# sekulas/vRod

Measured on AMD Instinct MI355X. Metric: queries/sec + recall@10 vs CPU ref, 10M×768 cosine, batch=1024, 1/2/4/8 GPU, higher is better.
Workload: dtype bf16

## Files before the change

vrod_amd/csrc/kernels_mfma_w4.hip:

```cpp
#include "mfma_common.h"
#include "w4_steal.h"

namespace vrod {

#ifdef VROD_W4_CLK
__device__ unsigned long long g_w4_clk[8];
#define W4_CLK(...) __VA_ARGS__
#else
#define W4_CLK(...)
#endif

template <int BASE, bool ZERO>
__device__ __forceinline__ void w4_mfma1(const bf16x8& x, const bf16x8& y) {
    if constexpr (ZERO)
        asm volatile("v_mfma_f32_16x16x32_bf16 a[%c2:%c3], %0, %1, 0" ::"v"(x), "v"(y), "i"(BASE), "i"(BASE + 3) : "memory");
    else
        asm volatile("v_mfma_f32_16x16x32_bf16 a[%c2:%c3], %0, %1, a[%c2:%c3]" ::"v"(x), "v"(y), "i"(BASE), "i"(BASE + 3) : "memory");
}
template <int MH, int NH, bool ZERO, int G>
__device__ __forceinline__ void w4_mfma_group(const bf16x8 (&FA)[4][2], const bf16x8 (&FB)[4][2]) {
    static_for<0, 4>([&](auto ic) {
        constexpr int I = G * 4 + decltype(ic)::value;
        constexpr int kk = I / 16, mm = (I / 4) % 4, nn = I % 4;
        w4_mfma1<((MH * 4 + mm) * 8 + NH * 4 + nn) * 4, ZERO && kk == 0>(FA[mm][kk], FB[nn][kk]);
    });
}
template <int BASE>
__device__ __forceinline__ f32x4 w4_read_acc() {
    f32x4 v;
    asm volatile("v_accvgpr_read_b32 %0, a[%c4]\n\tv_accvgpr_read_b32 %1, a[%c5]\n\tv_accvgpr_read_b32 %2, a[%c6]\n\tv_accvgpr_read_b32 %3, a[%c7]"
                 : "=v"(v[0]), "=v"(v[1]), "=v"(v[2]), "=v"(v[3]) : "i"(BASE), "i"(BASE + 1), "i"(BASE + 2), "i"(BASE + 3));
    return v;
}

#ifndef W4_RD_STRIDE_S
#define W4_RD_STRIDE_S "36"
#endif
__device__ __forceinline__ f32x4 w4_read_acc_dyn(uint32_t t) {
    f32x4 v;
    uint32_t tmp;
#define W4_RD(T)                                                                                    \
    "v_accvgpr_read_b32 %0, a[4*" #T "]\n\tv_accvgpr_read_b32 %1, a[4*" #T "+1]\n\t"                \
    "v_accvgpr_read_b32 %2, a[4*" #T "+2]\n\tv_accvgpr_read_b32 %3, a[4*" #T "+3]\n\ts_branch .Lw4rd_e_%=\n\t"
#define W4_RD8(A, B, C, D, E, F, G, H) W4_RD(A) W4_RD(B) W4_RD(C) W4_RD(D) W4_RD(E) W4_RD(F) W4_RD(G) W4_RD(H)
    asm volatile("s_getpc_b64 vcc\n"
                 ".Lw4rd_a_%=:\n\t"
                 "s_mul_i32 %4, %5, " W4_RD_STRIDE_S "\n\t"
                 "s_add_u32 vcc_lo, vcc_lo, %4\n\t"
                 "s_addc_u32 vcc_hi, vcc_hi, 0\n\t"
                 "s_add_u32 vcc_lo, vcc_lo, .Lw4rd_t_%=-.Lw4rd_a_%=\n\t"
                 "s_addc_u32 vcc_hi, vcc_hi, 0\n\t"
                 "s_setpc_b64 vcc\n"
                 ".Lw4rd_t_%=:\n\t"
                 W4_RD8(0, 1, 2, 3, 4, 5, 6, 7) W4_RD8(8, 9, 10, 11, 12, 13, 14, 15)
                 W4_RD8(16, 17, 18, 19, 20, 21, 22, 23) W4_RD8(24, 25, 26, 27, 28, 29, 30, 31)
                 W4_RD8(32, 33, 34, 35, 36, 37, 38, 39) W4_RD8(40, 41, 42, 43, 44, 45, 46, 47)
                 W4_RD8(48, 49, 50, 51, 52, 53, 54, 55) W4_RD8(56, 57, 58, 59, 60, 61, 62, 63)
                 ".Lw4rd_e_%=:"
                 : "=v"(v[0]), "=v"(v[1]), "=v"(v[2]), "=v"(v[3]), "=&s"(tmp)
                 : "s"(t)
                 : "vcc", "scc");
#undef W4_RD8
#undef W4_RD
    return v;
}

constexpr uint32_t kDumpEntryBytes = 128;
constexpr uint32_t kDumpWaveBytes = (kLdsTotalW4 - kLdsDump) / 4;
constexpr uint32_t kDumpCap = kDumpWaveBytes / (kDumpEntryBytes + 4);
static_assert(kDumpRegionBytes == kDumpRegionCap * (kDumpEntryBytes + 4), "spill region layout");
constexpr int kLdsNext = kLdsDump + kDumpCap * (kDumpEntryBytes + 4);
static_assert(kLdsNext % 8 == 0 && kLdsNext + 12 <= kLdsDump + (int)kDumpWaveBytes, "the claimed range sits in the slack of wave 0's log");
static_assert(kDumpCap >= 48 && kDumpCap * (kDumpEntryBytes + 4) <= kDumpWaveBytes && kDumpWaveBytes % 16 == 0, "hit dump layout");

template <int N>
__device__ __forceinline__ void w4_dump_column(uint32_t entry_addr , uint32_t desc_addr, uint32_t desc) {
    asm volatile("ds_write_b128 %0, a[%c3:%c4]\n\t"
                 "ds_write_b128 %0, a[%c5:%c6] offset:16\n\t"
                 "ds_write_b128 %0, a[%c7:%c8] offset:32\n\t"
                 "ds_write_b128 %0, a[%c9:%c10] offset:48\n\t"
                 "ds_write_b128 %0, a[%c11:%c12] offset:64\n\t"
                 "ds_write_b128 %0, a[%c13:%c14] offset:80\n\t"
                 "ds_write_b128 %0, a[%c15:%c16] offset:96\n\t"
                 "ds_write_b128 %0, a[%c17:%c18] offset:112\n\t"
                 "ds_write_b32 %1, %2"
                 :: "v"(entry_addr), "v"(desc_addr), "v"(desc),
                    "i"(N * 4), "i"(N * 4 + 3), "i"(N * 4 + 32), "i"(N * 4 + 35), "i"(N * 4 + 64), "i"(N * 4 + 67),
                    "i"(N * 4 + 96), "i"(N * 4 + 99), "i"(N * 4 + 128), "i"(N * 4 + 131), "i"(N * 4 + 160), "i"(N * 4 + 163),
                    "i"(N * 4 + 192), "i"(N * 4 + 195), "i"(N * 4 + 224), "i"(N * 4 + 227)
                 : "memory");
}

template <int METRIC>
__device__ __forceinline__ void w4_process_region(const MfmaKernelArgs& a, const float* thr_l, const float* qn2_l, const char* region,
                                                  uint32_t n_entries, uint32_t qb, int wr, int wc, int lane) {
    asm volatile("s_waitcnt vmcnt(0)" ::: "memory");
    const uint32_t* desc = reinterpret_cast<const uint32_t*>(region + kDumpRegionCap * kDumpEntryBytes);
    constexpr int kU = 4;
    const uint32_t nquads = n_entries * 8u;
#pragma unroll 1
    for (uint32_t base = 0; base < nquads; base += 64u * kU) {
        f32x4 v[kU];
        uint32_t d[kU];
#pragma unroll
        for (int u = 0; u < kU; ++u) {
            const uint32_t i = base + (uint32_t)u * 64u + (uint32_t)lane;
            const uint32_t ii = i < nquads ? i : 0u;
            v[u] = __builtin_nontemporal_load(reinterpret_cast<const f32x4*>(region + (ii >> 3) * kDumpEntryBytes + (ii & 7u) * 16u));
            d[u] = __builtin_nontemporal_load(desc + (ii >> 3));
        }
        uint32_t gq[kU], row0[kU], hits[kU], pos[kU];
        float sc[kU][4];
#pragma unroll
        for (int u = 0; u < kU; ++u) {
            const uint32_t i = base + (uint32_t)u * 64u + (uint32_t)lane;
            const uint32_t m = i & 7u;
            const uint32_t ln = d[u] & 63u, n = (d[u] >> 6) & 7u, tile = a.tile_first + (d[u] >> 9);
            const uint32_t ql = wc * 128 + n * 16 + (ln & 15u);
            gq[u] = qb * kBN + ql;
            row0[u] = tile * kBM + wr * 128 + m * 16 + (ln >> 4) * 4;
            const float thr = thr_l[ql];
            const float qn2 = METRIC == M_L2 ? qn2_l[ql] : 0.0f;
            uint32_t h = 0u;
#pragma unroll
            for (int r = 0; r < 4; ++r) {
                const uint32_t row = row0[u] + r;
                sc[u][r] = METRIC == M_COSINE ? v[u][r] : __builtin_fmaf(-2.0f, v[u][r], a.xnorm2[row] + qn2);
                h |= (better<METRIC>(sc[u][r], thr) && row >= a.row_lo && row < a.row_end) ? 1u << r : 0u;
            }
            hits[u] = i < nquads ? h : 0u;
        }
#pragma unroll
        for (int u = 0; u < kU; ++u) {
            pos[u] = 0u;
            if (hits[u]) pos[u] = atomicAdd(&a.counts[gq[u]], (uint32_t)__builtin_popcount(hits[u]));
        }
#pragma unroll
        for (int u = 0; u < kU; ++u)
#pragma unroll
            for (int r = 0; r < 4; ++r)
                if ((hits[u] >> r) & 1u) {
                    if (pos[u] < a.cap) a.lists[(uint64_t)gq[u] * a.cap + pos[u]] = make_uint2(__float_as_uint(sc[u][r]), row0[u] + r);
                    ++pos[u];
                }
    }
    __builtin_amdgcn_s_waitcnt(0x0F70);
}
template <int METRIC>
__device__ __forceinline__ void w4_spill(const MfmaKernelArgs& a, const float* thr_l, const float* qn2_l, const char* wlog_lds, uint32_t n,
                                         char* region, uint32_t& wglob, uint32_t qb, int wr, int wc, int lane) {
    asm volatile("s_waitcnt lgkmcnt(0)" ::: "memory");
    if (wglob + n > kDumpRegionCap) {
        w4_process_region<METRIC>(a, thr_l, qn2_l, region, wglob, qb, wr, wc, lane);
        wglob = 0u;
    }
    for (uint32_t i = lane; i < n * 8u; i += 64u)
        *reinterpret_cast<f32x4*>(region + (size_t)wglob * kDumpEntryBytes + i * 16u) = *reinterpret_cast<const f32x4*>(wlog_lds + i * 16u);
    if ((uint32_t)lane < n)
        reinterpret_cast<uint32_t*>(region + kDumpRegionCap * kDumpEntryBytes)[wglob + lane] =
            reinterpret_cast<const uint32_t*>(wlog_lds + kDumpCap * kDumpEntryBytes)[lane];
    wglob += n;
}

template <int METRIC>
__device__ __forceinline__ void w4_filter_tile(const MfmaKernelArgs& a, const float* thr_l, const float* qn2_l, const float* xn_l,
                                               uint32_t tile, uint32_t ql0, uint32_t qb, char* wlog_lds, char* region, int wr, int wc, int lane,
                                               uint32_t& wlog, uint32_t& wglob ) {
    float thr[8], qn2[8];
#pragma unroll
    for (int n = 0; n < 8; ++n) {
        thr[n] = thr_l[ql0 + n * 16];
        qn2[n] = METRIC == M_L2 ? qn2_l[ql0 + n * 16] : 0.0f;
    }
    asm volatile("s_nop 15\n\ts_nop 7" ::: "memory");
    float best[8];
#pragma unroll
    for (int n = 0; n < 8; ++n) best[n] = worst_score(METRIC);
    static_for<0, 8>([&](auto mc) {
        constexpr int m = decltype(mc)::value;
        f32x4 xv = f32x4{0.f, 0.f, 0.f, 0.f};
        if constexpr (METRIC == M_L2) xv = *reinterpret_cast<const f32x4*>(xn_l + m * 16);
        static_for<0, 8>([&](auto nc) {
            constexpr int n = decltype(nc)::value;
            const f32x4 v = w4_read_acc<(m * 8 + n) * 4>();
#pragma unroll
            for (int r = 0; r < 4; ++r) {
                const float sc = METRIC == M_COSINE ? v[r] : __builtin_fmaf(-2.0f, v[r], xv[r] + qn2[n]);
                best[n] = METRIC == M_COSINE ? __builtin_fmaxf(best[n], sc) : __builtin_fminf(best[n], sc);
            }
        });
    });
#ifdef VROD_W4_AUDIT_SELFTEST
    asm volatile("; selftest %0" :: "a"(best[0] + best[1]));
#endif
    uint32_t colmask = 0u, pend = 0u;
#pragma unroll
    for (int n = 0; n < 8; ++n) {
        const bool hl = better<METRIC>(best[n], thr[n]);
        pend |= hl ? 1u << n : 0u;
        colmask |= __any(hl) ? 1u << n : 0u;
    }
    
    if (colmask) {
        const uint32_t log_addr = (uint32_t)(uintptr_t)(__attribute__((address_space(3))) void*)wlog_lds;
        const uint32_t dword = ((tile - a.tile_first) << 9) | (uint32_t)lane;
#pragma unroll 1
        for (;;) {
            bool again = false;
            static_for<0, 8>([&](auto nc) {
                constexpr int n = decltype(nc)::value;
                if (!(colmask & (1u << n))) return;
                const bool hl = (pend >> n) & 1u;
                const unsigned long long hm = __ballot(hl);
                if (hm == 0ull) return;
                
                const uint32_t pos = wlog + __builtin_amdgcn_mbcnt_hi((uint32_t)(hm >> 32), __builtin_amdgcn_mbcnt_lo((uint32_t)hm, 0u));
                const bool fit = hl && pos < kDumpCap;
                if (fit) {
                    w4_dump_column<n>(log_addr + pos * kDumpEntryBytes, log_addr + kDumpCap * kDumpEntryBytes + pos * 4u, dword | ((uint32_t)n << 6));
                    pend &= ~(1u << n);
                }
                const unsigned long long fm = __ballot(fit);
                wlog += (uint32_t)__builtin_popcountll(fm);
                again |= fm != hm;
            });
            if (!again) break;
            w4_spill<METRIC>(a, thr_l, qn2_l, wlog_lds, wlog, region, wglob, qb, wr, wc, lane);
            wlog = 0u;
            
        }
        asm volatile("s_waitcnt lgkmcnt(0)" ::: "memory");
    }
    
}

template <int METRIC>
__device__ __forceinline__ void w4_dense_store_tile(const MfmaKernelArgs& a, const float* qn2_l, uint32_t ql0, uint32_t row_w, uint32_t gq0) {
    float qn2[8];
#pragma unroll
    for (int n = 0; n < 8; ++n) qn2[n] = METRIC == M_L2 ? qn2_l[ql0 + n * 16] : 0.0f;
    asm volatile("s_nop 15\n\ts_nop 7" ::: "memory");
    static_for<0, 8>([&](auto mc) {
        constexpr int m = decltype(mc)::value;
        const uint32_t row = row_w + m * 16;
        f32x4 xv = f32x4{0.f, 0.f, 0.f, 0.f};
        if constexpr (METRIC == M_L2) xv = *reinterpret_cast<const f32x4*>(a.xnorm2 + row);
        const bool in = row - a.row_lo < a.dense_ld;
        static_for<0, 8>([&](auto nc) {
            constexpr int n = decltype(nc)::value;
            const f32x4 v = w4_read_acc<(m * 8 + n) * 4>();
            f32x4 sc;
#pragma unroll
            for (int r = 0; r < 4; ++r) sc[r] = METRIC == M_COSINE ? v[r] : __builtin_fmaf(-2.0f, v[r], xv[r] + qn2[n]);
            if (in) *reinterpret_cast<f32x4*>(a.dense_out + (uint64_t)(gq0 + n * 16) * a.dense_ld + (row - a.row_lo)) = sc;
        });
    });
}

template <int METRIC>
__device__ __forceinline__ void w4_groupmax_store_tile(const MfmaKernelArgs& a, const float* qn2_l, const float* xn_l, uint32_t ql0,
                                                       uint32_t gq0, uint32_t group) {
    asm volatile("" : "+v"(gq0), "+v"(group));
    asm volatile("s_nop 15\n\ts_nop 7" ::: "memory");
    const uint32_t off0 = gq0 * a.dense_ld + group, step = 16u * a.dense_ld;
    static_for<0, 8>([&](auto nc) {
        constexpr int n = decltype(nc)::value;
        const float qn2 = METRIC == M_L2 ? qn2_l[ql0 + n * 16] : 0.0f;
        float best = worst_score(METRIC);
        static_for<0, 8>([&](auto mc) {
            constexpr int m = decltype(mc)::value;
            f32x4 xv = f32x4{0.f, 0.f, 0.f, 0.f};
            if constexpr (METRIC == M_L2) xv = *reinterpret_cast<const f32x4*>(xn_l + m * 16);
            const f32x4 v = w4_read_acc<(m * 8 + n) * 4>();
#pragma unroll
            for (int r = 0; r < 4; ++r) {
                const float sc = METRIC == M_COSINE ? v[r] : __builtin_fmaf(-2.0f, v[r], xv[r] + qn2);
                best = METRIC == M_COSINE ? __builtin_fmaxf(best, sc) : __builtin_fminf(best, sc);
            }
        });
        if (group < a.dense_ld) a.dense_out[off0 + (uint32_t)n * step] = best;
        __builtin_amdgcn_sched_barrier(0);
    });
}

template <int IMM>
__device__ __forceinline__ void w4_dma_piece(uint32_t lds_buf, uint32_t voff, const char* sbase) {
    asm volatile("s_add_u32 m0, %0, %c3\n\ts_nop 0\n\tglobal_load_lds_dwordx4 %1, %2" :: "s"(lds_buf), "v"(voff), "s"(sbase), "i"(IMM) : "scc", "memory");
}
template <int IMM>
__device__ __forceinline__ void w4_dma_m0(uint32_t lds_buf) {
    asm volatile("s_add_u32 m0, %0, %c1" :: "s"(lds_buf), "i"(IMM) : "scc", "memory");
}
__device__ __forceinline__ void w4_dma_load(uint32_t voff, const char* sbase) {
    asm volatile("global_load_lds_dwordx4 %0, %1" :: "v"(voff), "s"(sbase) : "memory");
}
__device__ __forceinline__ const char* w4_uniform_ptr(const char* p) {
    const uint64_t v = (uint64_t)p;
    const uint32_t lo = __builtin_amdgcn_readfirstlane((uint32_t)v), hi = __builtin_amdgcn_readfirstlane((uint32_t)(v >> 32));
    return (const char*)(((uint64_t)hi << 32) | lo);
}

__device__ __forceinline__ void w4_strip_range(const MfmaKernelArgs& a, uint32_t s, uint32_t& b, uint32_t& e) {
    b = a.tile_first + (uint32_t)((uint64_t)a.ntiles * s / a.nstrips);
    e = a.tile_first + (uint32_t)((uint64_t)a.ntiles * (s + 1) / a.nstrips);
}
__device__ __forceinline__ bool w4_claim(const MfmaKernelArgs& a, uint32_t strip, uint32_t qbl, uint32_t& own_next, int lane, uint32_t& cb, uint32_t& ce) {
    uint32_t* words = a.claims + qbl * a.nstrips;
    auto chunk = [&](uint32_t s, uint32_t j) {
        uint32_t b, e;
        w4_strip_range(a, s, b, e);
        w4_chunk_range(b, e, j, cb, ce);
    };
    {
        uint32_t b, e;
        w4_strip_range(a, strip, b, e);
        const uint32_t cpt = w4_tail_chunks(e - b);
        while (own_next < cpt) {
            const uint32_t j = own_next++;
            uint32_t old = 0u;
            if (lane == 0) old = atomicOr(&words[strip], 1u << j);
            old = __builtin_amdgcn_readfirstlane(old);
            if (!((old >> j) & 1u)) { chunk(strip, j); return true; }
        }
    }
    for (uint32_t base = 1u; base < a.nstrips; base += 64u) {
        const uint32_t v = base + (uint32_t)lane;
        const uint32_t s = (strip + v) % a.nstrips;
        uint32_t free_bits = 0u;
        if (v < a.nstrips) {
            uint32_t b, e;
            w4_strip_range(a, s, b, e);
            const uint32_t cpt = w4_tail_chunks(e - b);
            const uint32_t w = __hip_atomic_load(&words[s], __ATOMIC_RELAXED, __HIP_MEMORY_SCOPE_AGENT);
            free_bits = ~w & (cpt >= 32u ? 0xFFFFFFFFu : ((1u << cpt) - 1u));
        }
        unsigned long long cand = __ballot(free_bits != 0u);
        while (cand) {
            const int L = __builtin_ctzll(cand);
            uint32_t ok = 0u, jj = 0u;
            if (lane == L) {
                jj = 31u - (uint32_t)__builtin_clz(free_bits);
                const uint32_t old = atomicOr(&words[s], 1u << jj);
                ok = ((old >> jj) & 1u) ? 0u : 1u;
                free_bits &= ~(old | (1u << jj));
            }
            if (__builtin_amdgcn_readlane(ok, L)) {
                chunk(__builtin_amdgcn_readlane(s, L), __builtin_amdgcn_readlane(jj, L));
                return true;
            }
            cand = __ballot(free_bits != 0u);
        }
    }
    return false;
}

template <int METRIC, int DENSE, bool SPLIT>
__global__ __launch_bounds__(256) void scan_mfma_w4_kernel(const MfmaKernelArgs a) {
    extern __shared__ __attribute__((aligned(16))) char lds[];
    asm volatile("" ::: "a0", "a1", "a2", "a3", "a4", "a5", "a6", "a7", "a8", "a9", "a10", "a11", "a12", "a13", "a14", "a15", "a16", "a17", "a18", "a19", "a20", "a21", "a22", "a23", "a24", "a25", "a26", "a27", "a28", "a29", "a30", "a31", "a32", "a33", "a34", "a35", "a36", "a37", "a38", "a39", "a40", "a41", "a42", "a43", "a44", "a45", "a46", "a47", "a48", "a49", "a50", "a51", "a52", "a53", "a54", "a55", "a56", "a57", "a58", "a59", "a60", "a61", "a62", "a63", "a64", "a65", "a66", "a67", "a68", "a69", "a70", "a71", "a72", "a73", "a74", "a75", "a76", "a77", "a78", "a79", "a80", "a81", "a82", "a83", "a84", "a85", "a86", "a87", "a88", "a89", "a90", "a91", "a92", "a93", "a94", "a95", "a96", "a97", "a98", "a99", "a100", "a101", "a102", "a103", "a104", "a105", "a106", "a107", "a108", "a109", "a110", "a111", "a112", "a113", "a114", "a115", "a116", "a117", "a118", "a119", "a120", "a121", "a122", "a123", "a124", "a125", "a126", "a127", "a128", "a129", "a130", "a131", "a132", "a133", "a134", "a135", "a136", "a137", "a138", "a139", "a140", "a141", "a142", "a143", "a144", "a145", "a146", "a147", "a148", "a149", "a150", "a151", "a152", "a153", "a154", "a155", "a156", "a157", "a158", "a159", "a160", "a161", "a162", "a163", "a164", "a165", "a166", "a167", "a168", "a169", "a170", "a171", "a172", "a173", "a174", "a175", "a176", "a177", "a178", "a179", "a180", "a181", "a182", "a183", "a184", "a185", "a186", "a187", "a188", "a189", "a190", "a191", "a192", "a193", "a194", "a195", "a196", "a197", "a198", "a199", "a200", "a201", "a202", "a203", "a204", "a205", "a206", "a207", "a208", "a209", "a210", "a211", "a212", "a213", "a214", "a215", "a216", "a217", "a218", "a219", "a220", "a221", "a222", "a223", "a224", "a225", "a226", "a227", "a228", "a229", "a230", "a231", "a232", "a233", "a234", "a235", "a236", "a237", "a238", "a239", "a240", "a241", "a242", "a243", "a244", "a245", "a246", "a247", "a248", "a249", "a250", "a251", "a252", "a253", "a254", "a255");

    const int tid = threadIdx.x, lane = tid & 63;
    const int wave = __builtin_amdgcn_readfirstlane(tid >> 6);
    const int wr = wave >> 1, wc = wave & 1;
    uint32_t strip, qb0, qb_step;
    if (!wg_assignment(a, strip, qb0, qb_step)) return;
    const uint32_t t0 = a.tile_first + (uint32_t)((uint64_t)a.ntiles * strip / a.nstrips);
    const uint32_t t1 = a.tile_first + (uint32_t)((uint64_t)a.ntiles * (strip + 1) / a.nstrips);
    if (t0 >= t1) return;

    const uint32_t lds_addr = (uint32_t)(uintptr_t)(__attribute__((address_space(3))) void*)lds;
    char* wlog_lds = lds + kLdsDump + (uint32_t)wave * kDumpWaveBytes;
    char* region = a.dump + (size_t)(blockIdx.x * 4u + (uint32_t)wave) * kDumpRegionBytes;

    const uint32_t KT = a.ld_bytes >> 7;
    const uint32_t st_row = lane >> 3;
    const uint32_t lda_bytes = SPLIT ? a.lda_bytes : a.ld_bytes;
    const uint32_t st_lane_off_a = st_row * lda_bytes + (((lane & 7) ^ st_row) << 4);
    const uint32_t st_lane_off_b = st_row * a.ld_bytes + (((lane & 7) ^ st_row) << 4);
    const uint32_t fr = lane & 15, fg = lane >> 4, r7 = fr & 7;
    const uint32_t a_frag0 = ((wr * 16 + (fr >> 3)) << 10) + (r7 << 7);
    const uint32_t b_frag0 = 32768u + ((wc * 16 + (fr >> 3)) << 10) + (r7 << 7);
    const uint32_t c_off0 = ((0 * 4 + fg) ^ r7) << 4, c_off1 = ((1 * 4 + fg) ^ r7) << 4;
    const uint32_t piece_stride_a = 8u * lda_bytes, piece_stride_b = 8u * a.ld_bytes;
    const uint32_t t1s = (DENSE == 0 && a.claims != nullptr && KT >= 3u) ? t1 - w4_tail_tiles(t1 - t0) : t1;
    uint32_t total_it = 0xFFFFFFFFu;

    const uint32_t qb = a.qb_base + qb0;
    {
        float* thr_l = reinterpret_cast<float*>(lds + kLdsThr);
        float* qn2_l = reinterpret_cast<float*>(lds + kLdsQn2);
        const float* xn_l = reinterpret_cast<const float*>(lds + kLdsXn2);
        if (tid == 0) lds_zero3(reinterpret_cast<uint32_t*>(lds + kLdsNext));
        thr_l[tid] = DENSE ? 0.0f : a.thr[qb * kBN + tid];
        qn2_l[tid] = METRIC == M_L2 ? a.qnorm2[qb * kBN + tid] : 0.0f;
        const char* ua_src = w4_uniform_ptr(a.corpus + (uint64_t)t0 * kBM * lda_bytes);
        const char* ub_src = w4_uniform_ptr(a.queries + (uint64_t)qb * kBN * a.ld_bytes);
        const uint32_t p0 = ((uint32_t)wave >> 1) * 16u + ((uint32_t)wave & 1u) * 4u;
        uint32_t voa[8], vob[8];
#pragma unroll
        for (int j = 0; j < 8; ++j) {
            voa[j] = st_lane_off_a + (p0 + (uint32_t)(j & 3) + (uint32_t)(j >> 2) * 8u) * piece_stride_a;
            vob[j] = st_lane_off_b + (p0 + (uint32_t)(j & 3) + (uint32_t)(j >> 2) * 8u) * piece_stride_b;
        }
        const uint32_t lds_w = __builtin_amdgcn_readfirstlane(lds_addr + p0 * 1024u);
        uint32_t st_kt = 0, st_tile = t0, a_kt = 0;
        uint32_t st_end = t1s;
        bool pace_on = true;
        const uint32_t next_addr = (uint32_t)(uintptr_t)(__attribute__((address_space(3))) void*)(lds + kLdsNext);
#define W4_STAGE_A(BUF, H, I) w4_dma_piece<((I) + 8 * (H)) * 1024>(lds_w + ((BUF) & 1u) * kStageBytes, voa[(I) + 4 * (H)], ua_src);
#define W4_STAGE_B(BUF, H, I) w4_dma_piece<32768 + ((I) + 8 * (H)) * 1024>(lds_w + ((BUF) & 1u) * kStageBytes, vob[(I) + 4 * (H)], ub_src);
        auto stage_advance = [&](int32_t it_adv ) {
            if (st_kt + 1 < KT) {
                const bool hold = SPLIT && (st_kt % 3u) == 0u;
                if constexpr (SPLIT) a_kt += hold ? 0u : 1u;
                ua_src += hold ? 0 : 128;
                ub_src += 128;
                ++st_kt;
            } else {
                uint32_t nt = st_tile + 1u;
                bool have = nt < st_end;
                if (DENSE == 0 && !have) {
                    const uint2 nx = *reinterpret_cast<const uint2*>(lds + kLdsNext);
                    if (nx.y > nx.x) { nt = nx.x; st_end = nx.y; have = true; pace_on = false; }
                }
                if (have) {
                    const int64_t a_back = SPLIT ? (int64_t)a_kt * 128 : (int64_t)(KT - 1) * 128;
                    ua_src += (int64_t)(int32_t)(nt - st_tile) * ((int64_t)kBM * lda_bytes) - a_back;
                    ub_src -= (int64_t)(KT - 1) * 128;
                    if constexpr (SPLIT) a_kt = 0u;
                    st_kt = 0u;
                    st_tile = nt;
                    if (DENSE == 0 && nt + 1u == st_end && wave == 0 && t1s != t1) {
                        uint32_t cb = 0u, ce = 0u;
                        uint32_t own_next = *reinterpret_cast<const uint32_t*>(lds + kLdsNext + 8);
                        (void)w4_claim(a, strip, qb0, own_next, lane, cb, ce);
                        if (lane == 0)
                            asm volatile("ds_write_b64 %0, %1\n\tds_write_b32 %0, %2 offset:8\n\ts_waitcnt lgkmcnt(0)"
                                         :: "v"(next_addr), "v"(((uint64_t)ce << 32) | cb), "v"(own_next) : "memory");
                    }
                } else if (total_it == 0xFFFFFFFFu) {
                    total_it = (uint32_t)(it_adv + 3);
                }
            }
            ua_src = w4_uniform_ptr(ua_src);
            ub_src = w4_uniform_ptr(ub_src);
        };

#define W4_STAGE_UNIT(B) W4_STAGE_A(B, 0, 0) W4_STAGE_B(B, 0, 0) W4_STAGE_A(B, 0, 1) W4_STAGE_B(B, 0, 1) W4_STAGE_A(B, 0, 2) W4_STAGE_B(B, 0, 2)   \
                         W4_STAGE_A(B, 0, 3) W4_STAGE_B(B, 0, 3) W4_STAGE_A(B, 1, 0) W4_STAGE_B(B, 1, 0) W4_STAGE_A(B, 1, 1) W4_STAGE_B(B, 1, 1)   \
                         W4_STAGE_A(B, 1, 2) W4_STAGE_B(B, 1, 2) W4_STAGE_A(B, 1, 3) W4_STAGE_B(B, 1, 3)
        W4_STAGE_UNIT(0u)
        stage_advance(-2);
        W4_STAGE_UNIT(1u)
        stage_advance(-1);
#undef W4_STAGE_UNIT
        asm volatile("s_waitcnt vmcnt(0)" ::: "memory");
        __syncthreads();

        bf16x8 FA0[4][2], FA1[4][2], FBx[4][2], FBy[4][2];
#define W4_LOAD_A1(FA, MH, L, J) FA[(J) >> 1][(J) & 1] = *reinterpret_cast<const bf16x8*>((L) + a_frag0 + ((MH) * 4 + ((J) >> 1)) * 2048 + (((J) & 1) ? c_off1 : c_off0));
#define W4_LOAD_B1(FB, NH, L, J) FB[(J) >> 1][(J) & 1] = *reinterpret_cast<const bf16x8*>((L) + b_frag0 + ((NH) * 4 + ((J) >> 1)) * 2048 + (((J) & 1) ? c_off1 : c_off0));
#define W4_PHASE_S(FA, FB, MH, NH, ZERO, LD, DM)                                                   \
    __builtin_amdgcn_s_waitcnt(0xC07F);                                                            \
    DM(0, 0) w4_mfma_group<MH, NH, ZERO, 0>(FA, FB); LD(0) LD(1) DM(0, 1)                          \
    w4_mfma_group<MH, NH, ZERO, 1>(FA, FB); LD(2) LD(3) DM(1, 0)                                   \
    w4_mfma_group<MH, NH, ZERO, 2>(FA, FB); LD(4) LD(5) DM(1, 1)                                   \
    w4_mfma_group<MH, NH, ZERO, 3>(FA, FB); LD(6) LD(7) DM(2, 0)                                   \
    w4_mfma_group<MH, NH, ZERO, 4>(FA, FB); DM(2, 1)                                               \
    w4_mfma_group<MH, NH, ZERO, 5>(FA, FB); DM(3, 0)                                               \
    w4_mfma_group<MH, NH, ZERO, 6>(FA, FB); DM(3, 1)                                               \
    w4_mfma_group<MH, NH, ZERO, 7>(FA, FB);
#define W4_KTILE(BX, BY, LDQ0, LDQ3, ZERO)                                                         \
    W4_PHASE_S(FA0, BX, 0, 0, ZERO, LDQ0, W4_DMU0)                                                 \
    W4_PHASE_S(FA0, BY, 0, 1, ZERO, W4_LDQ1, W4_DMU1)                                              \
    asm volatile(W4_VMWAIT ::: "memory");                                                          \
    W4_LOOP_BARRIER();                                                                             \
    W4_PHASE_S(FA1, BY, 1, 1, ZERO, W4_LDQ2, W4_DMU2)                                              \
    W4_PHASE_S(FA1, BX, 1, 0, ZERO, LDQ3, W4_DMU3)
#ifdef VROD_W4_ABL_NODMA
#define W4_DMU0(j, L)
#define W4_DMU1(j, L)
#define W4_DMU2(j, L)
#define W4_DMU3(j, L)
#define W4_VMWAIT "s_waitcnt lgkmcnt(0)"
#else
#define W4_HALF_A(H, I, LOAD) if constexpr (LOAD) w4_dma_load(voa[(I) + 4 * (H)], ua_src); else w4_dma_m0<((I) + 8 * (H)) * 1024>(lds_wp);
#define W4_HALF_B(H, I, LOAD) if constexpr (LOAD) w4_dma_load(vob[(I) + 4 * (H)], ub_src); else w4_dma_m0<32768 + ((I) + 8 * (H)) * 1024>(lds_wp);
#define W4_DMU0(j, L) W4_HALF_A(0, j, L)
#define W4_DMU1(j, L) W4_HALF_B(0, j, L)
#define W4_DMU2(j, L) W4_HALF_B(1, j, L)
#define W4_DMU3(j, L) W4_HALF_A(1, j, L)
#define W4_VMWAIT "s_waitcnt vmcnt(16) lgkmcnt(0)"
#endif
#ifdef VROD_W4_ABL_NOEPI
#define W4_ABL_EPI false
#else
#define W4_ABL_EPI true
#endif
#ifdef VROD_W4_ABL_NOBAR
#define W4_LOOP_BARRIER()
#else
#define W4_LOOP_BARRIER() VROD_BARRIER()
#endif
#define W4_ITER(BX, BY, LDQ0, LDQ3, PAR)                                                           \
    {                                                                                              \
        const char* l = lds + (PAR) * kStageBytes;                                                 \
        const char* ln = lds + (1 - (PAR)) * kStageBytes;                                          \
        const uint32_t lds_wp = lds_w + (PAR) * kStageBytes;                                       \
        const bool first = kt == 0;                                                                \
                                                             \
           \
        if (--pace_left == 0u) {                                                                   \
          pace_left = a.pace_every;                                                                \
          ++pace_round;                                                                            \
          if (pace_on && tid == 0) {                                                               \
            uint32_t* ctr = a.pace + strip;                                                        \
            __hip_atomic_fetch_add(ctr, 1u, __ATOMIC_RELAXED, __HIP_MEMORY_SCOPE_AGENT);           \
            const uint32_t want = a.nqb * pace_round;                                              \
            bool ok = false;                                                                       \
                          \
            for (uint32_t spin = 0; spin < 64u; ++spin) {                                          \
                if (__hip_atomic_load(ctr, __ATOMIC_RELAXED, __HIP_MEMORY_SCOPE_AGENT) >= want) { ok = true; break; } \
                __builtin_amdgcn_s_sleep(2);                                                       \
            }                                                                                      \
            pace_on = ok;                                                                          \
          }                                                                                        \
        }                                                                                          \
              \
        if (METRIC == M_L2 && DENSE != 1 && first && wave == 0)                                    \
            w4_dma_piece<0>(lds_addr + kLdsXn2 + (tile & 1u) * 1024u, (uint32_t)lane * 16u, w4_uniform_ptr(reinterpret_cast<const char*>(a.xnorm2 + (uint64_t)tile * kBM))); \
        if (first) { W4_KTILE(BX, BY, LDQ0, LDQ3, true) } else { W4_KTILE(BX, BY, LDQ0, LDQ3, false) } \
        stage_advance((int32_t)it);                                                                \
        const bool last = kt == KT - 1;                                                            \
        W4_CLK(uint32_t ce1 = 0;)                                                                  \
        if (last) {                                                                                \
            W4_CLK(const uint32_t ce0 = (uint32_t)__builtin_amdgcn_s_memtime();)                   \
            if constexpr (DENSE == 2)                                                              \
                w4_groupmax_store_tile<METRIC>(a, qn2_l, xn_l + (tile & 1) * 256 + wr * 128 + fg * 4, wc * 128 + fr, \
                                               qb * kBN + wc * 128 + fr, ((tile - a.tile_first) * 2 + wr) * 4 + fg); \
            else if constexpr (DENSE == 1)                                                         \
                w4_dense_store_tile<METRIC>(a, qn2_l, wc * 128 + fr, tile * kBM + wr * 128 + fg * 4, qb * kBN + wc * 128 + fr); \
            else if (W4_ABL_EPI)                                                                   \
                w4_filter_tile<METRIC>(a, thr_l, qn2_l, xn_l + (tile & 1) * 256 + wr * 128 + fg * 4,        \
                                       tile, wc * 128 + fr, qb, wlog_lds, region, wr, wc, lane, wlog, wglob ); \
            W4_CLK(ce1 = (uint32_t)__builtin_amdgcn_s_memtime(); cke += ce1 - ce0; ckn += 1;)     \
            kt = 0;                                                                                \
            tile = KT >= 3u ? st_tile : tile + 1u;    \
        } else ++kt;                                                                               \
        asm volatile(W4_VMWAIT ::: "memory");                                                      \
        W4_LOOP_BARRIER();                                                                         \
        W4_CLK(if (last) ckb += (uint32_t)__builtin_amdgcn_s_memtime() - ce1;)                     \
        ++it;                                                                                      \
    }
#define W4_LDQ1(j) W4_LOAD_A1(FA1, 1, l, j)
#define W4_LDQ2(j) W4_LOAD_A1(FA0, 0, ln, j)
#define W4_LDQ0x(j) W4_LOAD_B1(FBy, 1, l, j)
#define W4_LDQ3x(j) W4_LOAD_B1(FBy, 0, ln, j)
#define W4_LDQ0y(j) W4_LOAD_B1(FBx, 1, l, j)
#define W4_LDQ3y(j) W4_LOAD_B1(FBx, 0, ln, j)
#define W4_LDP_A(j) W4_LOAD_A1(FA0, 0, lds, j)
#define W4_LDP_B(j) W4_LOAD_B1(FBx, 0, lds, j)
        W4_LDP_A(0) W4_LDP_A(1) W4_LDP_A(2) W4_LDP_A(3) W4_LDP_A(4) W4_LDP_A(5) W4_LDP_A(6) W4_LDP_A(7)
        W4_LDP_B(0) W4_LDP_B(1) W4_LDP_B(2) W4_LDP_B(3) W4_LDP_B(4) W4_LDP_B(5) W4_LDP_B(6) W4_LDP_B(7)
        asm volatile("s_waitcnt lgkmcnt(0)" ::: "memory");
        VROD_BARRIER();

        uint32_t it = 0, kt = 0, tile = t0;
        uint32_t wlog = 0u, wglob = 0u;
        uint32_t pace_left = a.pace_every ? a.pace_every + 1u : 0u, pace_round = 0u;
        
        W4_CLK(const uint64_t ck0 = __builtin_amdgcn_s_memtime(); const uint64_t cr0 = __builtin_amdgcn_s_memrealtime(); uint32_t cke = 0, ckb = 0, ckn = 0;)
        while (it < total_it) {
            W4_ITER(FBx, FBy, W4_LDQ0x, W4_LDQ3x, 0)
            if (it >= total_it) break;
            W4_ITER(FBy, FBx, W4_LDQ0y, W4_LDQ3y, 1)
        }
        
        W4_CLK(if (!DENSE && tid == 0) {
            const uint64_t ck1 = __builtin_amdgcn_s_memtime(), cr1 = __builtin_amdgcn_s_memrealtime();
            atomicAdd(&g_w4_clk[0], (unsigned long long)(ck1 - ck0)); atomicAdd(&g_w4_clk[1], (unsigned long long)(cr1 - cr0));
            atomicAdd(&g_w4_clk[2], 1ull); atomicAdd(&g_w4_clk[3], (unsigned long long)total_it);
            atomicAdd(&g_w4_clk[4], (unsigned long long)cke); atomicAdd(&g_w4_clk[5], (unsigned long long)ckb); atomicAdd(&g_w4_clk[6], (unsigned long long)ckn);
        })
#undef W4_LOAD_A1
#undef W4_LOAD_B1
#undef W4_PHASE_S
#undef W4_KTILE
#undef W4_VMWAIT
#undef W4_DMU0
#undef W4_DMU1
#undef W4_DMU2
#undef W4_DMU3
#undef W4_STAGE_A
#undef W4_STAGE_B
#undef W4_HALF_A
#undef W4_HALF_B
#undef W4_ITER
#undef W4_LDQ1
#undef W4_LDQ2
#undef W4_LDQ0x
#undef W4_LDQ3x
#undef W4_LDQ0y
#undef W4_LDQ3y
#undef W4_LDP_A
#undef W4_LDP_B
        asm volatile("s_waitcnt vmcnt(0)" ::: "memory");
        
        if constexpr (DENSE == 0) {
            if (wlog) w4_spill<METRIC>(a, thr_l, qn2_l, wlog_lds, wlog, region, wglob, qb, wr, wc, lane);
            if (wglob) w4_process_region<METRIC>(a, thr_l, qn2_l, region, wglob, qb, wr, wc, lane);
        }
        
        
    }
}

void launch_mfma_w4(const MfmaKernelArgs& a, int metric, int dense_form, bool split, int grid, hipStream_t s, hipEvent_t start, hipEvent_t stop) {
#define VROD_MFMA_W4K_(MM, DN, SP)                                                                          \
    do {                                                                                                    \
        static bool attr_set = false;                                                                       \
        if (!attr_set) {                                                                                    \
            (void)hipFuncSetAttribute((const void*)scan_mfma_w4_kernel<MM, DN, SP>,                         \
                                      hipFuncAttributeMaxDynamicSharedMemorySize, kLdsTotalW4);             \
            attr_set = true;                                                                                \
        }                                                                                                   \
        hipExtLaunchKernelGGL((scan_mfma_w4_kernel<MM, DN, SP>), dim3(grid), dim3(256), kLdsTotalW4, s, start, stop, 0, a); \
    } while (0)
#define VROD_MFMA_W4K(MM, DN) do { if (split) VROD_MFMA_W4K_(MM, DN, true); else VROD_MFMA_W4K_(MM, DN, false); } while (0)
#define VROD_MFMA_W4M(MM) do { if (dense_form == 0) VROD_MFMA_W4K(MM, 0); else if (dense_form == 2) VROD_MFMA_W4K(MM, 2); else VROD_MFMA_W4K(MM, 1); } while (0)
    if (metric == M_COSINE) VROD_MFMA_W4M(M_COSINE); else VROD_MFMA_W4M(M_L2);
#undef VROD_MFMA_W4M
#undef VROD_MFMA_W4K
#undef VROD_MFMA_W4K_
}

}


#ifdef VROD_W4_CLK
extern "C" int vrod_debug_w4_clk(unsigned long long* out8, int reset) {
    if (hipDeviceSynchronize() != hipSuccess) return -1;
    if (hipMemcpyFromSymbol(out8, HIP_SYMBOL(vrod::g_w4_clk), 8 * sizeof(unsigned long long)) != hipSuccess) return -1;
    if (reset) {
        unsigned long long z[8] = {};
        if (hipMemcpyToSymbol(HIP_SYMBOL(vrod::g_w4_clk), z, sizeof z) != hipSuccess) return -1;
    }
    return 0;
}
#endif
```

Before: 90300.

## Hand-schedule cosine filter epilogue with interleaved accvgpr reads and max3

```diff
diff --git a/vrod_amd/csrc/kernels_mfma_w4.hip b/vrod_amd/csrc/kernels_mfma_w4.hip
--- a/vrod_amd/csrc/kernels_mfma_w4.hip
+++ b/vrod_amd/csrc/kernels_mfma_w4.hip
@@ -162,34 +162,94 @@
     wglob += n;
 }
 
+#define W4E_R4(B, J, T)                                                                                       \
+    "v_accvgpr_read_b32 %[t" #B #J "0], a[(" #T ")*4]\n\tv_accvgpr_read_b32 %[t" #B #J "1], a[(" #T ")*4+1]\n\t"  \
+    "v_accvgpr_read_b32 %[t" #B #J "2], a[(" #T ")*4+2]\n\tv_accvgpr_read_b32 %[t" #B #J "3], a[(" #T ")*4+3]\n\t"
+#define W4E_M0(B, J, N, FIRST) "v_max3_f32 %[b" #N "], %[t" #B #J "0], " FIRST(N) ", %[t" #B #J "1]\n\t"
+#define W4E_M1(B, J, N) "v_max3_f32 %[b" #N "], %[b" #N "], %[t" #B #J "2], %[t" #B #J "3]\n\t"
+#define W4E_CONT(N) "%[b" #N "]"
+#define W4E_INIT(N) "%[ninf]"
+#define W4E_STEP(B, M, N0, P, Q0, Q1, Q2, Q3, S)                                                              \
+    W4E_R4(B, 0, M * 8 + N0 + 0) W4E_M0(P, 0, Q0, S)                                                          \
+    W4E_R4(B, 1, M * 8 + N0 + 1) W4E_M0(P, 1, Q1, S)                                                          \
+    W4E_R4(B, 2, M * 8 + N0 + 2) W4E_M0(P, 2, Q2, S) W4E_M0(P, 3, Q3, S)                                      \
+    W4E_R4(B, 3, M * 8 + N0 + 3) W4E_M1(P, 0, Q0) W4E_M1(P, 1, Q1)                                           \
+    W4E_M1(P, 2, Q2) W4E_M1(P, 3, Q3)
+#define W4E_MAXONLY(P, Q0, Q1, Q2, Q3)                                                                        \
+    W4E_M0(P, 0, Q0, W4E_CONT) W4E_M0(P, 1, Q1, W4E_CONT) W4E_M0(P, 2, Q2, W4E_CONT) W4E_M0(P, 3, Q3, W4E_CONT) \
+    W4E_M1(P, 0, Q0) W4E_M1(P, 1, Q1) W4E_M1(P, 2, Q2) W4E_M1(P, 3, Q3)
+#define W4E_CMP(N, D) "v_cmp_gt_f32_e64 %[" #D "], %[b" #N "], %[h" #N "]\n\t"
+
+__device__ __forceinline__ uint64_t w4_colmax_cos(const float (&thr)[8], float (&best)[8]) {
+    float x[16], y[16];
+    uint64_t hit, tmp;
+    asm volatile(
+        W4E_R4(x, 0, 0) W4E_R4(x, 1, 1) W4E_R4(x, 2, 2) W4E_R4(x, 3, 3)
+        W4E_STEP(y, 1, 0, x, 0, 1, 2, 3, W4E_INIT)
+        W4E_STEP(x, 2, 0, y, 0, 1, 2, 3, W4E_CONT) W4E_STEP(y, 3, 0, x, 0, 1, 2, 3, W4E_CONT)
+        W4E_STEP(x, 0, 4, y, 0, 1, 2, 3, W4E_CONT)
+        W4E_STEP(y, 1, 4, x, 4, 5, 6, 7, W4E_INIT)
+        W4E_STEP(x, 2, 4, y, 4, 5, 6, 7, W4E_CONT) W4E_STEP(y, 3, 4, x, 4, 5, 6, 7, W4E_CONT)
+        W4E_STEP(x, 4, 4, y, 4, 5, 6, 7, W4E_CONT) W4E_STEP(y, 5, 4, x, 4, 5, 6, 7, W4E_CONT)
+        W4E_STEP(x, 6, 4, y, 4, 5, 6, 7, W4E_CONT) W4E_STEP(y, 7, 4, x, 4, 5, 6, 7, W4E_CONT)
+        W4E_STEP(x, 4, 0, y, 4, 5, 6, 7, W4E_CONT) W4E_STEP(y, 5, 0, x, 0, 1, 2, 3, W4E_CONT)
+        W4E_STEP(x, 6, 0, y, 0, 1, 2, 3, W4E_CONT) W4E_STEP(y, 7, 0, x, 0, 1, 2, 3, W4E_CONT)
+        W4E_MAXONLY(y, 0, 1, 2, 3)
+        W4E_CMP(4, hit) W4E_CMP(5, tmp) "s_or_b64 %[hit], %[hit], %[tmp]\n\t"
+        W4E_CMP(6, tmp) "s_or_b64 %[hit], %[hit], %[tmp]\n\t" W4E_CMP(7, tmp) "s_or_b64 %[hit], %[hit], %[tmp]\n\t"
+        W4E_CMP(0, tmp) "s_or_b64 %[hit], %[hit], %[tmp]\n\t" W4E_CMP(1, tmp) "s_or_b64 %[hit], %[hit], %[tmp]\n\t"
+        W4E_CMP(2, tmp) "s_or_b64 %[hit], %[hit], %[tmp]\n\t" W4E_CMP(3, tmp) "s_or_b64 %[hit], %[hit], %[tmp]"
+        : [b0] "=&v"(best[0]), [b1] "=&v"(best[1]), [b2] "=&v"(best[2]), [b3] "=&v"(best[3]),
+          [b4] "=&v"(best[4]), [b5] "=&v"(best[5]), [b6] "=&v"(best[6]), [b7] "=&v"(best[7]),
+          [tx00] "=&v"(x[0]), [tx01] "=&v"(x[1]), [tx02] "=&v"(x[2]), [tx03] "=&v"(x[3]),
+          [tx10] "=&v"(x[4]), [tx11] "=&v"(x[5]), [tx12] "=&v"(x[6]), [tx13] "=&v"(x[7]),
+          [tx20] "=&v"(x[8]), [tx21] "=&v"(x[9]), [tx22] "=&v"(x[10]), [tx23] "=&v"(x[11]),
+          [tx30] "=&v"(x[12]), [tx31] "=&v"(x[13]), [tx32] "=&v"(x[14]), [tx33] "=&v"(x[15]),
+          [ty00] "=&v"(y[0]), [ty01] "=&v"(y[1]), [ty02] "=&v"(y[2]), [ty03] "=&v"(y[3]),
+          [ty10] "=&v"(y[4]), [ty11] "=&v"(y[5]), [ty12] "=&v"(y[6]), [ty13] "=&v"(y[7]),
+          [ty20] "=&v"(y[8]), [ty21] "=&v"(y[9]), [ty22] "=&v"(y[10]), [ty23] "=&v"(y[11]),
+          [ty30] "=&v"(y[12]), [ty31] "=&v"(y[13]), [ty32] "=&v"(y[14]), [ty33] "=&v"(y[15]),
+          [hit] "=&s"(hit), [tmp] "=&s"(tmp)
+        : [ninf] "s"(-__builtin_huge_valf()),
+          [h0] "v"(thr[0]), [h1] "v"(thr[1]), [h2] "v"(thr[2]), [h3] "v"(thr[3]),
+          [h4] "v"(thr[4]), [h5] "v"(thr[5]), [h6] "v"(thr[6]), [h7] "v"(thr[7])
+        : "scc");
+    return hit;
+}
+#undef W4E_R4
+#undef W4E_M0
+#undef W4E_M1
+#undef W4E_CONT
+#undef W4E_INIT
+#undef W4E_STEP
+#undef W4E_MAXONLY
+#undef W4E_CMP
+
 template <int METRIC>
 __device__ __forceinline__ void w4_filter_tile(const MfmaKernelArgs& a, const float* thr_l, const float* qn2_l, const float* xn_l,
-                                               uint32_t tile, uint32_t ql0, uint32_t qb, char* wlog_lds, char* region, int wr, int wc, int lane,
+                                               const float (&thr)[8], const float (&qn2)[8],
+                                               uint32_t tile, uint32_t qb, char* wlog_lds, char* region, int wr, int wc, int lane,
                                                uint32_t& wlog, uint32_t& wglob ) {
-    float thr[8], qn2[8];
-#pragma unroll
-    for (int n = 0; n < 8; ++n) {
-        thr[n] = thr_l[ql0 + n * 16];
-        qn2[n] = METRIC == M_L2 ? qn2_l[ql0 + n * 16] : 0.0f;
-    }
-    asm volatile("s_nop 15\n\ts_nop 7" ::: "memory");
     float best[8];
-#pragma unroll
-    for (int n = 0; n < 8; ++n) best[n] = worst_score(METRIC);
-    static_for<0, 8>([&](auto mc) {
-        constexpr int m = decltype(mc)::value;
-        f32x4 xv = f32x4{0.f, 0.f, 0.f, 0.f};
-        if constexpr (METRIC == M_L2) xv = *reinterpret_cast<const f32x4*>(xn_l + m * 16);
-        static_for<0, 8>([&](auto nc) {
-            constexpr int n = decltype(nc)::value;
-            const f32x4 v = w4_read_acc<(m * 8 + n) * 4>();
-#pragma unroll
-            for (int r = 0; r < 4; ++r) {
-                const float sc = METRIC == M_COSINE ? v[r] : __builtin_fmaf(-2.0f, v[r], xv[r] + qn2[n]);
-                best[n] = METRIC == M_COSINE ? __builtin_fmaxf(best[n], sc) : __builtin_fminf(best[n], sc);
-            }
+    if constexpr (METRIC == M_COSINE) {
+        if (!w4_colmax_cos(thr, best)) return;
+    } else {
+#pragma unroll
+        for (int n = 0; n < 8; ++n) best[n] = worst_score(METRIC);
+        static_for<0, 4>([&](auto qc) {
+            constexpr int q = decltype(qc)::value, mh = q / 2, nh = q == 1 || q == 2;
+            static_for<0, 4>([&](auto mc) {
+                constexpr int m = mh * 4 + decltype(mc)::value;
+                const f32x4 xv = *reinterpret_cast<const f32x4*>(xn_l + m * 16);
+                static_for<0, 4>([&](auto nc) {
+                    constexpr int n = nh * 4 + decltype(nc)::value;
+                    const f32x4 v = w4_read_acc<(m * 8 + n) * 4>();
+#pragma unroll
+                    for (int r = 0; r < 4; ++r) best[n] = __builtin_fminf(best[n], __builtin_fmaf(-2.0f, v[r], xv[r] + qn2[n]));
+                });
+            });
         });
-    });
+    }
 #ifdef VROD_W4_AUDIT_SELFTEST
     asm volatile("; selftest %0" :: "a"(best[0] + best[1]));
 #endif
@@ -200,7 +260,7 @@
         pend |= hl ? 1u << n : 0u;
         colmask |= __any(hl) ? 1u << n : 0u;
     }
-    
+
     if (colmask) {
         const uint32_t log_addr = (uint32_t)(uintptr_t)(__attribute__((address_space(3))) void*)wlog_lds;
         const uint32_t dword = ((tile - a.tile_first) << 9) | (uint32_t)lane;
@@ -229,7 +289,6 @@
             wlog = 0u;
             
         }
-        asm volatile("s_waitcnt lgkmcnt(0)" ::: "memory");
     }
     
 }
@@ -541,8 +600,8 @@
             else if constexpr (DENSE == 1)                                                         \
                 w4_dense_store_tile<METRIC>(a, qn2_l, wc * 128 + fr, tile * kBM + wr * 128 + fg * 4, qb * kBN + wc * 128 + fr); \
             else if (W4_ABL_EPI)                                                                   \
-                w4_filter_tile<METRIC>(a, thr_l, qn2_l, xn_l + (tile & 1) * 256 + wr * 128 + fg * 4,        \
-                                       tile, wc * 128 + fr, qb, wlog_lds, region, wr, wc, lane, wlog, wglob ); \
+                w4_filter_tile<METRIC>(a, thr_l, qn2_l, xn_l + (tile & 1) * 256 + wr * 128 + fg * 4, thr_r, qn2_r, \
+                                       tile, qb, wlog_lds, region, wr, wc, lane, wlog, wglob ); \
             W4_CLK(ce1 = (uint32_t)__builtin_amdgcn_s_memtime(); cke += ce1 - ce0; ckn += 1;)     \
             kt = 0;                                                                                \
             tile = KT >= 3u ? st_tile : tile + 1u;    \
@@ -567,6 +626,12 @@
 
         uint32_t it = 0, kt = 0, tile = t0;
         uint32_t wlog = 0u, wglob = 0u;
+        float thr_r[8], qn2_r[8];
+#pragma unroll
+        for (int n = 0; n < 8; ++n) {
+            thr_r[n] = DENSE == 0 ? thr_l[wc * 128 + fr + n * 16] : 0.0f;
+            qn2_r[n] = DENSE == 0 && METRIC == M_L2 ? qn2_l[wc * 128 + fr + n * 16] : 0.0f;
+        }
         uint32_t pace_left = a.pace_every ? a.pace_every + 1u : 0u, pace_round = 0u;
         
         W4_CLK(const uint64_t ck0 = __builtin_amdgcn_s_memtime(); const uint64_t cr0 = __builtin_amdgcn_s_memrealtime(); uint32_t cke = 0, ckb = 0, ckn = 0;)
```

Result: no change. 91050 (median of 6 runs) (+0.8%).
